# ishovkun/poroelasticity-dealii

Hardware: AMD Instinct MI355X
Metric: DoF-updates/sec in assemble+SpMV per fixed-stress iter (higher is better)
Workload: dtype f64

## Files before the change

poroelasticity_dealii_amd/csrc/common.hpp:

```cpp
#pragma once
#include <hip/hip_runtime.h>
#include <cstdint>
#include <cstdio>
#include <map>
#include <memory>
#include <type_traits>
#include <stdexcept>
#include <string>
#include <list>
#include <vector>
#include "../../include/poroel_hip.h"
#include "fdm_tables.hpp"
#include "cell_field.hpp"

namespace poro {

#define PORO_HIP(x)                                                                                   \
  do { hipError_t e_ = (x); if (e_ != hipSuccess) throw poro::Error(std::string(#x) + " -> " + hipGetErrorString(e_)); } while (0)

template <class T> struct DevBuf {
  T *p = nullptr; size_t n = 0;
  DevBuf() = default; DevBuf(const DevBuf &) = delete; DevBuf &operator=(const DevBuf &) = delete;
  ~DevBuf() { release(); }
  void release() { if (p) (void)hipFree(p); p = nullptr; n = 0; }
// ... 319 lines not shown
void p_residual_stencil(hipStream_t s, int dim, const BoxDev &box, double kappa, const double *t, const double *p, const double *src, double *R);
void p_stencil_apply_var(hipStream_t s, int dim, const BoxDev &box, double a, const double *kap, int ncomp, const double *x, double *y);
void p_residual_stencil_var(hipStream_t s, int dim, const BoxDev &box, const double *kap, int ncomp, const double *t, const double *p, const double *src, double *R);

struct KronCheb { const double *g = nullptr; double *znew = nullptr; double omega = 0; const uint8_t *cls = nullptr; const double *tab = nullptr;
                  double *side_lo = nullptr, *side_hi = nullptr; };
bool kron_supported(int dim, int k_u);
void kron_prepare_device();
BoxCoupling box_coupling(int dim, int k_u, const BoxDev &box);
void box_rhs_u(hipStream_t s, int dim, const BoxCoupling &B, double alpha, const double *p, const double *lift, const double *neu, const uint8_t *mask, double *rhs,
               const uint8_t *flags = nullptr );
int64_t box_rhs_u_flag_count(int64_t n_u);
void box_rhs_u_flags(hipStream_t s, const double *lift, const double *neu, int64_t n_u, uint8_t *flags );
void box_asm_u_matrix(hipStream_t s, int dim, int k_u, const BoxDev &box, const double *Ke, const CsrDev &A, const uint8_t *mask, double *val);
void box_proj_rhs(hipStream_t s, int dim, const BoxCoupling &B, const double *u, int n_comp, const int32_t *tensor_components, double *const *rhs);
void fdm_window_batch(hipStream_t s, double *grid, double *dense, double *dense_self, int self, bool to_block, const FdmWindow *win, int n_peers, int n_planes_pad, int64_t C, int64_t grid_stride, int64_t blk);
void fdm_window(hipStream_t s, double *dst, const double *src, bool to_block, int n_planes, int n_planes_pad, int64_t C, int64_t ncols_valid, int64_t grid_stride, int64_t grid_col0, int64_t grid_plane0);
void fdm_transform(hipStream_t s, const double *T, int n_l, int64_t SI, int64_t n_outer, const double *in, double *out, const FdmScale *scale);
void q1_line_factor(hipStream_t s, int dim, int nw, const FdmScalar &F, int nl, double a, const double *coef, double *inv);
void q1_line_solve(hipStream_t s, int dim, int nw, const FdmScalar &F, int nl, double a, bool fixed_lo, bool fixed_hi, const double *coef, const double *inv, const double *in, double *out);
void fdm_apply(hipStream_t s, const FdmScalar &F, double a, const double k[3], const double *g, double *z, double *t1, double *t2);
void fdmu_upload_dir(FdmuDir &D, const LineTables &T, bool single, bool split);
void fdmu_apply(hipStream_t s, const FdmU &F, const double *g, double *z, void *t1, void *t2, int stage);
void fdmu_window(hipStream_t s, double *dst, const double *src, bool to_block, int ncomp, int n_planes, int n_planes_pad, int64_t C, int64_t ncols_valid,
                 int64_t grid_stride, int64_t grid_planes, int64_t grid_col0, int64_t grid_plane0);
void fdmu_lines(hipStream_t s, const FdmU &F, const FdmuDir *last_dir, int64_t C, int64_t col0, int64_t ncol_valid, void *in, void *out);
struct FdmuLineArgs { int nl, n0; int64_t ncol; const double *coef; const double *lam0[3], *lam1[3]; int fixed[3][2]; };
void fdmu_line_factor(hipStream_t s, int ku, int ncomp, const FdmuLineArgs &a, double *fac );
void fdmu_line_solve(hipStream_t s, int ku, int ncomp, const FdmuLineArgs &a, const double *fac, double *v );
bool fdmo_usable(int dim, const int nn[3]);
void fdmo_init(FdmOct &O, const int nn[3], const double coef[3][3], hipStream_t s);
void fdmo_init_slab(FdmOct &O, const int nn[3], const double coef[3][3], int rank, const std::vector<int> &node_layers, bool has_upper, hipStream_t s);
void fdmo_init_per_direction(FdmOct &O, const int nn[3], const double coef[3][3], const FdmFormDecision &D, hipStream_t s);
void fdmo_upload_dir(FdmOct &O, int comp, int dir, const LineTables &T);
void fdmo_finalize(FdmOct &O);
void fdmo_apply(hipStream_t s, const FdmOct &O, const double *g_oct, double *z_oct, double *scratch_oct, const PcgScalars *gate = nullptr, hipEvent_t *ev  = nullptr,
                double *gz_part  = nullptr,
                int precision  = PORO_FDM_FP64,
                const PcgStopTest &stop = PcgStopTest{} );
bool fdmo_scalar_usable(int dim, const int nn[3]);
void fdmo_scalar_init(FdmOct &O, const int nn[3], hipStream_t s);
void fdmo_scalar_upload_dir(FdmOct &O, int dir, const LineTables &T);
void fdmo_scalar_apply(hipStream_t s, FdmOct &O, double a, double kappa, const double *g, double *z, const PcgScalars *gate = nullptr);
void fdmo_scalar_apply_many(hipStream_t s, FdmOct &O, double a, double kappa, int nb, const double *const *g, double *const *z, const PcgScalars *gate = nullptr);
void la_residual_norms_many(hipStream_t s, int nb, const double *const *y, const double *const *b, int64_t n, double *partials, const uint8_t *mask = nullptr);
void fdmo_scalar_init_slab(FdmOct &O, const int nn[3], int rank, const std::vector<int> &node_layers, hipStream_t s);
void fdmo_scalar_slab_pass(hipStream_t s, FdmOct &O, int pass, double a, double kappa, const double *in, double *out);
bool fdmo_planar_usable(int dim, const int nn[3]);
void fdmo_init_planar(FdmOct &O, const int nn[3], const double coef[3][3], hipStream_t s, bool split = true );
void fdmo_upload_dir_planar(FdmOct &O, int comp, int dir, const LineTables &T);
void fdmo_apply_planar(hipStream_t s, const FdmOct &O, const double *g_q, double *z_q, const PcgScalars *gate = nullptr, const PcgStopTest &stop = PcgStopTest{} );
void fdmo_from_nodal(hipStream_t s, const FdmOct &O, const double *v_nodal, double *q_oct);
void fdmo_to_nodal(hipStream_t s, const FdmOct &O, const double *r_oct, double *v_nodal);
void fdmo_init_residual(hipStream_t s, const FdmOct &O, double *g_oct, const double *Ax, const double *b, const uint8_t *inert);
void fdmo_first_direction(hipStream_t s, const FdmOct &O, double *d, const double *g_oct, const double *z_oct, double *partials );
void fdmo_update_g(hipStream_t s, const FdmOct &O, PcgScalars *sc, int parity, double *g_oct, const double *h, const uint8_t *inert, const double *partials_dh, double *partials_out , const double *red = nullptr);
void fdmo_update_d(hipStream_t s, const FdmOct &O, PcgScalars *sc, int parity, int it, double *x, double *d, const double *z_oct, const double *partials_in , const double *red = nullptr,
                   bool gz_from_pass = false ,
                   bool stream_x = false ,
                   bool decided = false ,
                   bool gg_stored = false );
void fdmo_dot_owned(hipStream_t s, const FdmOct &O, const double *a_oct, const double *b_oct, double *partials, const PcgScalars *gate);
void fdmo_slab_pass(hipStream_t s, const FdmOct &O, int pass , const double *in, double *out, const PcgScalars *gate, hipEvent_t e0 = nullptr, hipEvent_t e1 = nullptr);
void fdmo_slab_scatter_pack(hipStream_t s, const FdmOct &O, const PcgScalars *gate);
int kron_apply(hipStream_t s, const MfArgs &a, const double *x, double *y, bool constrained, int n_cus, double *dot_partials = nullptr, hipEvent_t ev0 = nullptr, hipEvent_t ev1 = nullptr,
               const PcgScalars *pcg = nullptr ,
               const KronCheb *cheb = nullptr );
void kron_fix_constrained(hipStream_t s, const MfArgs &a, const double *x, double *y, double *dot_partials, int slot_base);
void kron_lm_prepare_device();
int kron_lm_apply(hipStream_t s, const MfArgs &a, const double *planes, const double *x, double *y, bool constrained, int n_cus, double *dot_partials = nullptr, hipEvent_t ev0 = nullptr,
                  hipEvent_t ev1 = nullptr, const PcgScalars *pcg = nullptr);
void hyb_gather(hipStream_t s, int dim, int64_t n_box_nodes, const int64_t *inj, const double *x, double *x_box);
struct HybCombine { int64_t n_box_nodes, n_removed, n_chunks; const int64_t *inj; const uint8_t *touched; const int32_t *removed_cells, *slot, *chunk_cls; const int64_t *nodes;
                    const double *x_box, *y_box; double *V; };
void hyb_combine(hipStream_t s, const MfArgs &box, const double *Ke_t, bool constrained, const HybCombine &h, double *y);

}
```

poroelasticity_dealii_amd/csrc/ctx.hip:

```cpp
#include <dlfcn.h>
#include <rccl/rccl.h>
#include <algorithm>
#include <array>
#include <chrono>
#include <cmath>
#include <cstdlib>
#include <cstring>
#include <functional>
#include <thread>
#include <unordered_map>
#include "common.hpp"
#include "ctx_internal.hpp"

using namespace poro;
using namespace poro::ctx_detail;

namespace {
void lifting_from_wh(poro_ctx *c) {
  la_fill(c->stream, c->lift_u.p, 0.0, c->n_u);
  la_axpy(c->stream, c->lift_u.p, -1.0, c->wh_u.p, c->n_u);
}

void throw_unless_close(poro_ctx *c, double *a, const double *b, int64_t n, double rel_tol, const char *what) {
  hipStream_t s = c->stream;
// ... 204 lines not shown
        exchange_planes(c, c->cheb_side_lo.p, c->cheb_side_hi.p, plane);
      }
      la_cheb_fix_planes(s, zn, zj, g, kc.side_lo, c->comm.recv_lo.p, kc.side_hi, c->comm.recv_hi.p, sys.diag, omega, c->n_u, plane);
    }
    if (dp) la_dot_partials(s, g, zn, n_own, dp);
    return dp != nullptr;
  };
  auto step_fused = [&](const double *g, double *zj, double *zn, double omega, double *dp, const PcgScalars *pstate) {
    const KronCheb kc = cheb_update(g, zn, omega);
    if (dp) PORO_HIP(hipMemsetAsync(dp, 0, kMaxPartials * sizeof(double), s));
    const int slots = fused_kernel(zj, kc, dp, pstate);
    return dp && slots > 0;
  };
  auto step_unfused = [&](const double *g, double *zj, double *zn, double omega, double *dp) {
    sys.apply(zj, c->cheb_t.p, nullptr);
    la_cheb_step(s, zn, zj, g, c->cheb_t.p, sys.diag, omega, c->n_u, n_own, dp);
    return dp != nullptr;
  };
  sys.prec.z = z_u(c);
  sys.prec.gated = fuse;
  sys.prec.applications = m;
  sys.z1.out = (m % 2 == 0) ? sys.prec.z : c->cheb_z.p;
  sys.z1.scale = 1.0 / roots[0];
  sys.prec.fn = [&](const double *g, double *z, const PrecCall &call) {
    Timed tm(c, "precondition_u_chebyshev");
    double *X[2] = {(m % 2 == 0) ? z : c->cheb_z.p, (m % 2 == 0) ? c->cheb_z.p : z};
    if (!call.z1_ready) la_cheb_first(s, X[0], g, sys.diag, 1.0 / roots[0], c->n_u);
    bool dot_done = false;
    for (int j = 1; j <= m; ++j) {
      const double omega = 1.0 / roots[j];
      double *zj = X[(j - 1) & 1], *zn = X[j & 1];
      double *dp = j == m ? call.gz_partials : nullptr;
      if (fuse_multi) dot_done = step_fused_slabs(g, zj, zn, omega, dp);
      else if (fuse) dot_done = step_fused(g, zj, zn, omega, dp, call.gate);
      else dot_done = step_unfused(g, zj, zn, omega, dp);
      ++c->cheb_applies;
    }
    return dot_done ? GzLeft::in_partials : GzLeft::nowhere;
  };
  const int rc = pcg(c, sys, opts, info);
  finish_u(c, true);
  return rc;
}

int solve_u_fdm(poro_ctx *c, const poro_solver_opts *opts, poro_solve_info *info) {
  build_fdm_u(c);
  const FdmOct *oct = c->fdm_oct.built ? &c->fdm_oct : nullptr;
  const bool separate_gz = std::getenv("PORO_FDMO_SEPARATE_GZ") != nullptr;
  const bool shared = oct && !oct->slab.on && !oct->planar && std::getenv("PORO_FDMO_SEPARATE_BUFFERS") == nullptr;
  if (shared) c->timers["fdm_u_shared_buffers"].enqueued++;
  if (oct && oct->per_dir) c->timers["fdm_u_per_direction_form"].enqueued++;
  const int precision = oct && oct->per_dir ? PORO_FDM_FP64 : c->fdm_precision;
  double *const scratch = shared && precision != PORO_FDM_FP32 ? nullptr : c->fdm_oct.t.p;
  KrylovSystem sys = krylov_u(c, c->dir_mask.p, false, c->pcg_hint_fdm_u);
  if (shared) sys.h = c->fdm_oct.z.p;
  sys.oct.form = oct;
  sys.oct.stream_x = shared;
  sys.prec.z = c->wz_u.p;
  sys.prec.gated = oct != nullptr;
  sys.prec.decides_stop = oct && !oct->slab.on;
  sys.prec.fn = [&](const double *g, double *z, const PrecCall &call) {
    if (!oct) {
      fdm_precondition_u(c, g, z);
      return GzLeft::nowhere;
    }
    const bool gz = call.gz_partials && !separate_gz;
    return fdm_precondition_u_form(c, g, z, call.gate, precision, scratch, gz ? c->fdm_oct.gz_part.p : nullptr, call.stop) ? GzLeft::in_octant_form : GzLeft::nowhere;
  };
  const int rc = pcg(c, sys, opts, info);
  finish_u(c, false);
  return rc;
}

int solve_u_two_level(poro_ctx *c, const poro_solver_opts *opts, poro_solve_info *info) {
  if (!two_level_supported(c)) throw Error("PORO_PREC_TWO_LEVEL needs poro_desc.coarse (a refinement of a uniform box whose Dirichlet conditions cover whole faces)");
  const double om = opts->omega > 0 ? opts->omega : 1.0;
  KrylovSystem sys = krylov_u(c, c->cons_u.inert.p, false, c->pcg_hint_u);
  sys.prec.z = z_u(c);
  sys.prec.fn = [&](const double *g, double *z, const PrecCall &) {
    two_level_precondition_u(c, g, z, om);
    return GzLeft::nowhere;
  };
  const int rc = pcg(c, sys, opts, info);
  finish_u(c, true);
  return rc;
}

int solve_u_jacobi(poro_ctx *c, const poro_solver_opts *opts, poro_solve_info *info) {
  const int rc = pcg(c, krylov_u(c, c->cons_u.inert.p, true, c->pcg_hint_u), opts, info);
  finish_u(c, true);
  return rc;
}

struct Q1System {
  double a, kappa;
  const double *val;
  const double *dinv;
  DevBuf<double> *ilu;
  bool *ilu_valid;
  double *x;
  const double *b;
  int *hint;
  const uint8_t *inert;
  const uint8_t *inert_fdm = nullptr;
  Q1Set set = Q1Set::free_ends;
  Q1Set coarse_set = Q1Set::free_ends;
  const double *kap = nullptr;
  int kap_ncomp = 0;
  int perm_kind = 0;
  bool distribute_inhom = true;
// ... 806 lines not shown
```

poroelasticity_dealii_amd/csrc/ctx_internal.hpp:

```cpp
#pragma once
#include <rccl/rccl.h>
#include <functional>
#include <string>
#include <vector>
#include "common.hpp"
#include "whole_faces.hpp"
#include "fdm_tables.hpp"

namespace poro {
namespace ctx_detail {

extern thread_local std::string g_err;
inline int ipow(int b, int e) { int r = 1; while (e--) r *= b; return r; }
template <class F> int guarded(F &&f) {
  try { return f(); }
  catch (const std::exception &e) { g_err = e.what(); return -1; }
}
template <class F> void for_each_colour(poro_ctx *c, F &&fn) {
  for (size_t k = 0; k + 1 < c->color_off.size(); ++k)
    fn(c->color_cells.p + c->color_off[k], c->color_off[k + 1] - c->color_off[k]);
}

struct Rccl {
  void *lib = nullptr;
// ... 34 lines not shown
  ~EventPair() { c->event_pool.push_back(e0); c->event_pool.push_back(e1); }
  EventPair(const EventPair &) = delete; EventPair &operator=(const EventPair &) = delete;
};
void post_and_wait(poro_ctx *c, const double *dev_src, int n, const PcgScalars *sc = nullptr);

void setup_general_partition(poro_ctx *c, const poro_desc *d);
void exchange_planes(poro_ctx *c, const double *send_lo, const double *send_hi, int64_t plane);
void exchange_add(poro_ctx *c, double *v, int64_t n, int64_t plane);
void allreduce_sum(poro_ctx *c, double *dev, int n);
void allreduce_sum_vec(poro_ctx *c, double *dev, int64_t n, const char *timer);
int64_t owned(poro_ctx *c, int64_t n, int64_t plane);
AsmArgs asm_args(poro_ctx *c);
MfArgs mf_args(poro_ctx *c);
void mf_operator(poro_ctx *c, const double *x, double *y, bool constrained);
void mfg_operator(poro_ctx *c, const double *x, double *y, bool constrained);
void build_spatial_cells(poro_ctx *c);
void sync_moduli_planes(poro_ctx *c);
void hybrid_enable(poro_ctx *c);
void hybrid_operator(poro_ctx *c, const double *x, double *y, bool constrained);
void count_mfg_launches(poro_ctx *c, int n);
double *vec(poro_ctx *c, int which);
int64_t vec_len(poro_ctx *c, int which);
bool is_u_vec(int which);
bool apply_A_u(poro_ctx *c, const double *x, double *y, int mode, double *dot_partials = nullptr, bool fix_rows = true, const PcgScalars *pcg_state = nullptr,
               bool exchange = true );

typedef std::function<bool(const double *x, double *y, double *dh_partials)> ApplyFn;
struct PrecCall {
  const PcgScalars *gate = nullptr;
  double *gz_partials = nullptr;
  bool z1_ready = false;
  PcgStopTest stop;
};
enum class GzLeft { nowhere, in_partials , in_octant_form  };
typedef std::function<GzLeft(const double *g, double *z, const PrecCall &)> PrecFn;

struct KrylovSystem {
  int64_t n = 0, plane = 0;
  double *x = nullptr; const double *b = nullptr;
  ApplyFn apply;
  DiagVec diag;
  const uint8_t *inert = nullptr;
  double *g = nullptr, *d = nullptr, *h = nullptr;
  int cg1_set = 0;
  int *hint = nullptr;
  struct { PrecFn fn;
           double *z = nullptr;
           bool gated = false;
           bool decides_stop = false;
           int applications = 0;
  } prec;
  struct { const FdmOct *form = nullptr;
           bool stream_x = false;
  } oct;
  struct { double *out = nullptr; double scale = 0; } z1;
};
int pcg(poro_ctx *c, const KrylovSystem &sys, const poro_solver_opts *opts, poro_solve_info *info);
double dot_host(poro_ctx *c, const double *a, const double *b, int64_t n);
int pcg_csr_sweeps(poro_ctx *c, CsrDev &A, const double *val, DevBuf<double> &lu, bool &lu_valid, KrylovSystem &sys, const poro_solver_opts *opts, poro_solve_info *info);
double estimate_lmax_u(poro_ctx *c, const KrylovSystem &sys);

bool fdm_p_supported(poro_ctx *c);
bool fdm_pj_supported(poro_ctx *c);
enum class Q1Set { free_ends, fixed_ends };
inline FdmQ1 &q1_set(poro_ctx *c, Q1Set which) { return which == Q1Set::fixed_ends ? c->q1_fixed : c->q1_free; }
void build_fdm_q1(poro_ctx *c, Q1Set which);
int slab_layout(poro_ctx *c, SlabLayout &L, int nodes_per_cell, int64_t ncol_total);
const char *prec_refusal(poro_ctx *c, int which_system, int prec, bool solving = false);
void alltoall_blocks(poro_ctx *c, double *send, double *recv, int64_t blk, bool self_in_place = false );
void setup_two_level(poro_ctx *c, const poro_desc *d);
bool two_level_supported(poro_ctx *c);
bool two_level_supported_p(poro_ctx *c);
bool two_level_supported_pj(poro_ctx *c);
void two_level_precondition_p(poro_ctx *c, double a, double kappa, const double *dinv, const double *g, double *z, double omega, const uint8_t *inert, Q1Set coarse_set = Q1Set::free_ends);
void two_level_precondition_u(poro_ctx *c, const double *g, double *z, double omega);
bool fdm_precondition_u_form(poro_ctx *c, const double *g_form, double *z_form, const PcgScalars *gate, int precision, double *scratch, double *gz_part = nullptr, const PcgStopTest &stop = PcgStopTest{});
void fdm_precondition_u_nodal(poro_ctx *c, const double *g, double *z, int precision);
void fdm_precondition_p(poro_ctx *c, double a, const double k[3], const double *g, double *z, Q1Set which = Q1Set::free_ends);
void fdm_precondition_p_layered(poro_ctx *c, double a, const double *g, double *z, Q1Set which = Q1Set::free_ends);
void analyse_fdm_u(poro_ctx *c);
void build_fdm_u(poro_ctx *c);
FdmuLineArgs fdmu_line_args(poro_ctx *c);
void release_fdm_u(poro_ctx *c);
void fdm_precondition_u(poro_ctx *c, const double *g, double *z);

void validate_rows(const int64_t *ptr, const int32_t *col, const double *weight, int64_t n_rows, int64_t n_cols, const std::string &what);
void build_kelly_tables(poro_ctx *c);

void setup(poro_ctx *c, const poro_desc *d);
void sync_source_vector(poro_ctx *c);

}
}
```

poroelasticity_dealii_amd/csrc/ctx_pcg.hip:

```cpp
#include <dlfcn.h>
#include <rccl/rccl.h>
#include <algorithm>
#include <array>
#include <chrono>
#include <cmath>
#include <cstdlib>
#include <cstring>
#include <functional>
#include <thread>
#include <unordered_map>
#include "common.hpp"
#include "ctx_internal.hpp"

using namespace poro;
using namespace poro::ctx_detail;

namespace poro {
namespace ctx_detail {
static int expected_iterations(const int *hint, bool cheap_overshoot) {
  if (!hint || hint[0] <= 0) return 0;
  const int expect = std::max(hint[1] > 0 ? 2 * hint[0] - hint[1] : hint[0], hint[0] / 2);
  return std::min(expect, cheap_overshoot ? hint[0] + std::max(2, hint[0] / 4) : hint[0]);
}
template <class State> static int finish_solve(const KrylovSystem &sys, const State &hs, int64_t own, double seconds, poro_solve_info *info) {
// ... 13 lines not shown
  double *x = sys.x, *g = sys.g, *d = sys.d, *sv = sys.h, *w = wbuf.p, *z = precond ? sys.prec.z : zbuf.p;
  if (!z) throw Error("pcg: explicit preconditioner without a z vector");
  const bool jacobi = opts->preconditioner == PORO_PREC_JACOBI;
  Cg1State *st = c->cg1_state.p; double *part = c->partials.p, *red = c->red.p;
  EventPair ev(c); PORO_HIP(hipEventRecord(ev.e0, s));
  sys.apply(x, w, nullptr);
  pcg_init_residual(s, g, w, sys.b, sys.inert, n);
  la_fill(s, d, 0.0, n); la_fill(s, sv, 0.0, n);
  double *z1_out = sys.z1.out; double z1_scale = sys.z1.scale;
  if (jacobi && !precond) { z1_out = z; z1_scale = 1.0; }
  Cg1State hs{};
  int enq = 0;
  const int expect = expected_iterations(sys.hint, false);
  auto next_batch = [&](int done_its) { const int left = expect - 4 - done_its; return left >= 4 ? std::min(32, left) : 2; };
  int batch = expect > 0 ? next_batch(0) : 1;
  while (true) {
    for (int k = 0; k < batch; ++k) {
      if (precond) { PrecCall call; call.z1_ready = enq > 0 && sys.z1.out != nullptr; (void)precond(g, z, call); }
      else if (jacobi) { if (enq == 0) la_cheb_first(s, z, g, sys.diag, 1.0, n); }
      else la_copy(s, z, g, n);
      sys.apply(z, w, nullptr);
      cg1_dots(s, g, z, w, enq == 0 ? sys.b : nullptr, n_own, part);
      pcg_scalars_sum(s, part, 4, red);
      allreduce_sum(c, red, 4);
      cg1_scalars(s, st, red, enq == 0 ? 1 : 0, opts->abs_tol, opts->rel_tol, opts->max_iter, opts->stop_rule);
      cg1_update(s, st, d, sv, x, g, z, w, sys.diag, sys.inert, z1_out, z1_scale, n);
      ++enq;
    }
    PORO_HIP(hipMemcpyAsync(&hs, st, sizeof(hs), hipMemcpyDeviceToHost, s)); PORO_HIP(hipStreamSynchronize(s));
    if (hs.done) break;
    if (expect > 0) batch = next_batch(enq); else if (batch < 8) batch *= 2;
  }
  PORO_HIP(hipEventRecord(ev.e1, s)); PORO_HIP(hipEventSynchronize(ev.e1));
  float ms = 0; PORO_HIP(hipEventElapsedTime(&ms, ev.e0, ev.e1));
  return finish_solve(sys, hs, hs.it + 2, ms * 1e-3, info);
}

int pcg(poro_ctx *c, const KrylovSystem &sys, const poro_solver_opts *opts, poro_solve_info *info) {
  static const bool two_reductions = std::getenv("PORO_TWO_REDUCTION_CG") != nullptr;
  const FdmOct *oct = sys.oct.form;
  const bool multi = c->comm.multi();
  if (multi && !two_reductions && !oct) return pcg_single_reduction(c, sys, opts, info);
  hipStream_t s = c->stream;
  const PrecFn &precond = sys.prec.fn;
  const int prec = opts->preconditioner == PORO_PREC_JACOBI ? 1 : 0;
  if (oct && (!precond || multi != oct->slab.on)) throw Error("pcg: the octant form needs an explicit preconditioner (one rank: octants, slab partition: quadrants)");
  const int64_t n = sys.n, n_own = owned(c, n, sys.plane);
  double *x = sys.x, *d = sys.d, *h = sys.h, *g = oct ? oct->g.p : sys.g, *zbuf = oct ? oct->z.p : sys.prec.z;
  if (precond && !zbuf) throw Error("pcg: explicit preconditioner without a z vector");
  double *part = c->partials.p, *red = c->red.p; PcgScalars *sc = c->scal.p;
  double *part_dh = part + 3 * (size_t)kMaxPartials;
  const auto t_start = std::chrono::steady_clock::now();
  sys.apply(x, h, nullptr);
  if (oct) fdmo_init_residual(s, *oct, g, h, sys.b, sys.inert); else pcg_init_residual(s, g, h, sys.b, sys.inert, n);
  if (opts->stop_rule != PORO_STOP_REDUCTION) la_dot_partials(s, sys.b, sys.b, n_own, part);
  if (precond) (void)precond(g, zbuf, PrecCall{});
  if (oct) fdmo_first_direction(s, *oct, d, g, zbuf, part + kMaxPartials); else pcg_first_direction(s, d, g, sys.diag, zbuf, prec, n, n_own, part + kMaxPartials);
  pcg_scalars_sum(s, part, 3, red);
  allreduce_sum(c, red, 3);
  pcg_scalars_start(s, sc, red, opts->abs_tol, opts->rel_tol, opts->max_iter, opts->stop_rule);
  PORO_HIP(hipMemsetAsync(part_dh, 0, kMaxPartials * sizeof(double), s));
  PcgScalars hs{};
  int it = 0;
  const bool cheap_overshoot = !precond || sys.prec.gated;
  const int expect = expected_iterations(sys.hint, cheap_overshoot);
  const bool small = n <= 400000;
  int batch = expect > 0 ? (cheap_overshoot ? std::min(expect, 256) : std::max(1, expect - 1)) : (precond && !cheap_overshoot && !small ? 1 : 4);
  PrecCall call;
  call.gate = sys.prec.gated ? sc : nullptr; call.gz_partials = part + kMaxPartials; call.z1_ready = sys.z1.out != nullptr;
  const bool stop_in_prec = oct && !multi && sys.prec.gated && sys.prec.decides_stop && std::getenv("PORO_PCG_FINAL_PREC") == nullptr;
  const int stop_per_wave = std::getenv("PORO_PCG_STOP_PER_WAVE") != nullptr ? 1 : 0;
  const bool gg_stored = stop_in_prec && std::getenv("PORO_PCG_GG_RESUM") == nullptr;
  while (true) {
    for (int k = 0; k < batch; ++k) {
      ++it;
      if (stop_in_prec) call.stop = PcgStopTest{sc, part, it, stop_per_wave};
      if (!sys.apply(d, h, part_dh)) pcg_dot_dh(s, sc, d, h, n_own, part_dh);
      if (multi) { pcg_scalars_sum(s, part_dh, 1, red); allreduce_sum(c, red, 1); }
      if (oct) fdmo_update_g(s, *oct, sc, (it - 1) & 1, g, h, sys.inert, part_dh, part, multi ? red : nullptr);
      else pcg_update_g_fused(s, sc, (it - 1) & 1, g, h, sys.diag, zbuf, sys.z1.out, sys.z1.scale, prec, n, n_own, part_dh, multi ? red : nullptr, part);
      const GzLeft gz = precond ? precond(g, zbuf, call) : GzLeft::in_partials;
      if (gz == GzLeft::nowhere) {
        if (oct && multi) fdmo_dot_owned(s, *oct, g, zbuf, call.gz_partials, call.gate);
        else la_dot_partials(s, g, zbuf, oct ? oct->n_oct : n_own, call.gz_partials, call.gate);
      }
      if (multi) { pcg_scalars_sum(s, part, 2, red + 1); allreduce_sum(c, red + 1, 2); }
      if (oct) fdmo_update_d(s, *oct, sc, (it - 1) & 1, it, x, d, zbuf, part, multi ? red + 1 : nullptr, gz == GzLeft::in_octant_form, sys.oct.stream_x, stop_in_prec, gg_stored);
      else pcg_update_d_fused(s, sc, (it - 1) & 1, it, x, d, g, sys.diag, zbuf, prec, n, part, multi ? red + 1 : nullptr);
    }
    post_and_wait(c, nullptr, 0, sc); hs = c->mailbox->sc;
    if (hs.done || hs.finishing) break;
    if (expect > 0) batch = cheap_overshoot ? 3 : small ? 2 : 1;
    else if (cheap_overshoot && precond) batch = 4;
    else if (batch < 32) batch *= 2;
  }
  if (hs.stop) c->timers["fdm_u_final_prec_skipped"].enqueued++;
  return finish_solve(sys, hs, hs.it + 1, std::chrono::duration<double>(std::chrono::steady_clock::now() - t_start).count(), info);
}

void build_ssor_levels(poro_ctx *c, CsrDev &A) {
  if (A.ssor.built) return;
  std::vector<int64_t> rp(A.n + 1); std::vector<int32_t> col(A.nnz);
  PORO_HIP(hipMemcpy(rp.data(), A.rp.p, (A.n + 1) * sizeof(int64_t), hipMemcpyDeviceToHost)); PORO_HIP(hipMemcpy(col.data(), A.col.p, A.nnz * sizeof(int32_t), hipMemcpyDeviceToHost));
  auto levels = [&](bool fwd, DevBuf<int32_t> &rows_dev, std::vector<int64_t> &off) {
    std::vector<int32_t> lvl(A.n, 0); int maxl = 0;
    if (fwd) for (int64_t r = 0; r < A.n; ++r) { int l = 0; for (int64_t j = rp[r]; j < rp[r + 1] && col[j] < r; ++j) l = std::max(l, lvl[col[j]] + 1); lvl[r] = l; maxl = std::max(maxl, l); }
    else for (int64_t r = A.n - 1; r >= 0; --r) { int l = 0; for (int64_t j = rp[r + 1] - 1; j >= rp[r] && col[j] > r; --j) l = std::max(l, lvl[col[j]] + 1); lvl[r] = l; maxl = std::max(maxl, l); }
    off.assign(maxl + 2, 0);
    for (int64_t r = 0; r < A.n; ++r) off[lvl[r] + 1]++;
    for (int l = 0; l <= maxl; ++l) off[l + 1] += off[l];
    std::vector<int32_t> rows(A.n); std::vector<int64_t> pos(off.begin(), off.end() - 1);
    for (int64_t r = 0; r < A.n; ++r) rows[pos[lvl[r]]++] = (int32_t)r;
    rows_dev.upload(rows);
  };
  levels(true, A.ssor.fwd_rows, A.ssor.fwd_off); levels(false, A.ssor.bwd_rows, A.ssor.bwd_off);
  A.ssor.built = true;
}
double dot_host(poro_ctx *c, const double *a, const double *b, int64_t n) {
  la_dot_partials(c->stream, a, b, n, c->partials.p); la_reduce_finish(c->stream, c->partials.p, 1, c->red.p, 0);
  allreduce_sum(c, c->red.p, 1);
  post_and_wait(c, c->red.p, 1);
  return c->mailbox->vals[0];
}
static int pcg_host(poro_ctx *c, const KrylovSystem &sys, const poro_solver_opts *opts, poro_solve_info *info) {
  hipStream_t s = c->stream;
  const int64_t n = sys.n, n_own = n;
  double *x = sys.x, *g = sys.g, *d = sys.d, *h = sys.h; const double *b = sys.b;
  const auto t0 = std::chrono::steady_clock::now();
  int64_t applies = 0; int it = 0, conv = 0;
  sys.apply(x, g, nullptr); ++applies;
  la_axpy(s, g, -1.0, b, n);
  double res = std::sqrt(dot_host(c, g, g, n_own)); const double res0 = res;
  const double tol = std::max(opts->abs_tol, opts->rel_tol * (opts->stop_rule == PORO_STOP_REDUCTION ? res0 : std::sqrt(dot_host(c, b, b, n_own))));
  if (res <= tol) conv = 1;
  else {
    (void)sys.prec.fn(g, h, PrecCall{});
    la_fill(s, d, 0.0, n); la_axpy(s, d, -1.0, h, n);
    double gh = dot_host(c, g, h, n_own);
    while (true) {
      ++it;
// ... 81 lines not shown
```

poroelasticity_dealii_amd/csrc/kernels_fdmo.hip:

```cpp
#include "common.hpp"
#include "fdm_tables.hpp"
#include "device_reduce.hpp"
#include <hip/hip_ext.h>
#include <cmath>
#include <cstdlib>
#include <limits>
#include <mutex>
#include <set>
#include <type_traits>

namespace poro {
namespace {

typedef double v4d __attribute__((ext_vector_type(4)));
typedef float v4f __attribute__((ext_vector_type(4)));

struct OctDims { int nx, ny, nz, hx, hy, hz, hxp; int64_t co; int no, own_z, nc; int split; int part[8]; };

__device__ __forceinline__ void bfly_fwd(double (&v)[8], const bool (&centre)[3]) {
#pragma unroll
  for (int bit = 0; bit < 3; ++bit) {
    const int m = 1 << bit;
#pragma unroll
    for (int i = 0; i < 8; ++i) if (!(i & m)) {
// ... 116 lines not shown
  const double alpha = sc->gh2[parity] / dh;
  double gg = 0;
  for (int64_t t_ = (int64_t)blockIdx.x * kBlock + threadIdx.x; t_ < NC * (D.co / 2); t_ += (int64_t)gridDim.x * kBlock) {
    const int64_t pr = t_ / NC; const int c = (int)(t_ - NC * pr); const int64_t idx = 2 * pr;
    const OctPos<PD> P0(D, idx), P1(D, idx + 1);
    double w0[8], w1[8];
    const bool on0 = P0.valid && !(inert && inert[P0.node[0] * NC + c]), on1 = P1.valid && !(inert && inert[P1.node[0] * NC + c]);
#pragma unroll
    for (int m = 0; m < 8; ++m) { w0[m] = on0 ? h[P0.node[m] * NC + c] : 0.0; w1[m] = on1 ? h[P1.node[m] * NC + c] : 0.0; }
    bfly_fwd(w0, P0.centre); bfly_fwd(w1, P1.centre);
    double s0 = 0, s1 = 0;
#pragma unroll
    for (int o = 0; o < 8; ++o) if (part_on<PD>(D, o)) {
      double2 *gp = reinterpret_cast<double2 *>(g + (int64_t)(c * D.no + part_at<PD>(D, o)) * D.co + idx);
      double2 gv = *gp;
      gv.x = fma(alpha, w0[o], gv.x); gv.y = fma(alpha, w1[o], gv.y);
      *gp = gv; s0 = fma(gv.x, gv.x, s0); s1 = fma(gv.y, gv.y, s1);
    }
    if (P0.own) gg = fma(P0.weight, s0, fma(P1.weight, s1, gg));
  }
  gg = block_sum(gg, sh);
  store_partial(partials_out, gg);
  if (blockIdx.x == 0 && threadIdx.x == 0) { sc->dh = dh; sc->alpha = alpha; }
}
template <int NC, bool XNT, bool PD> __global__ void __launch_bounds__(kBlock) k_fdmo_update_d(OctDims D, PcgScalars *sc, int parity, int it, double *__restrict__ x, double *__restrict__ d, const double *__restrict__ z, int64_t n_u, const double *partials_in, const double *red,
                                                                            const double *gz_part, int gz_n, int decided ) {
  __shared__ double sh[5];
  if (sc->done) return;
  const double gg = red ? red[0] : decided == 2 ? sc->gg : sum_partials(partials_in, sh);
  const double res = sqrt(gg), gh_old = sc->gh2[parity], alpha = sc->alpha;
  const int stop = decided ? sc->stop : res <= sc->tol ? 1 : it >= sc->max_iter ? 2 : 0;
  const bool conv = stop == 1, fail = stop == 2, no_z = decided && stop;
  const double gz = no_z ? 0.0 : red ? red[1] : gz_part ? sum_partials(gz_part, sh, gz_n) : sum_partials(partials_in + kMaxPartials, sh);
  if (blockIdx.x == 0 && threadIdx.x == 0) { sc->gg = gg; if (!no_z) sc->gz = gz; sc->res = res; sc->it = it; }
  if (conv || fail) {
    for (int64_t i = (int64_t)blockIdx.x * kBlock + threadIdx.x; i < n_u; i += (int64_t)gridDim.x * kBlock) x[i] = fma(alpha, d[i], x[i]);
    if (blockIdx.x == 0 && threadIdx.x == 0) { sc->converged = conv ? 1 : 0; sc->finishing = 1; }
    return;
  }
  const double beta = gz / gh_old;
  PORO_OCT_LOOP(D) {
    PORO_OCT_DECODE(D)
    double w[8];
#pragma unroll
    for (int o = 0; o < 8; ++o) w[o] = part_on<PD>(D, o) ? z[(int64_t)(c * D.no + part_at<PD>(D, o)) * D.co + idx] : 0.0;
    bfly_bwd(w, P.centre);
#pragma unroll
    for (int m = 0; m < 8; ++m) if (P.live[m]) {
      const int64_t dof = P.node[m] * NC + c;
      const double dv = d[dof], xv = XNT ? __builtin_nontemporal_load(&x[dof]) : x[dof];
      if (XNT) __builtin_nontemporal_store(fma(alpha, dv, xv), &x[dof]); else x[dof] = fma(alpha, dv, xv);
      d[dof] = fma(beta, dv, -w[m]);
    }
  }
  if (blockIdx.x == 0 && threadIdx.x == 0) { sc->beta = beta; sc->gh2[parity ^ 1] = gz; }
}

__global__ void __launch_bounds__(kBlock) k_fdmo_dot_owned(OctDims D, const double *__restrict__ a, const double *__restrict__ b, double *partials, const PcgScalars *gate) {
  __shared__ double sh[5];
  if (gate && (gate->done | gate->finishing)) return;
  const int64_t per = (int64_t)D.own_z * D.hxp * D.hy;
  const int nblk = D.nc * D.no, share = gridDim.x / nblk, blk = blockIdx.x / max(share, 1), sub = blockIdx.x - blk * share;
  double acc = 0;
  if (share > 0 && blk < nblk) {
    const double2 *__restrict__ a2 = reinterpret_cast<const double2 *>(a + blk * D.co), *__restrict__ b2 = reinterpret_cast<const double2 *>(b + blk * D.co);
    for (int64_t e = (int64_t)sub * kBlock + threadIdx.x; e < per / 2; e += (int64_t)share * kBlock) { const double2 u = a2[e], v = b2[e]; acc = fma(u.x, v.x, fma(u.y, v.y, acc)); }
  }
  acc = block_sum(acc, sh);
  store_partial(partials, acc);
}

struct SlabGeo { int cw, nchunk, cps, chunk_total, rank, my_chunks, hzg, ng, np; int64_t scols, pl, co; };
__global__ void __launch_bounds__(256) k_fdmo_slab_scatter_pack(SlabGeo S, int rows, const int64_t *__restrict__ row_out, const int32_t *__restrict__ row_kz,
                                                                  const double *__restrict__ tz, double *__restrict__ buf, const PcgScalars *gate) {
  if (gate && (gate->done | gate->finishing)) return;
  const int per_row = S.my_chunks * S.cw, total = rows * per_row;
  for (int e = blockIdx.x * 256 + threadIdx.x; e < total; e += gridDim.x * 256) {
    const int row = e / per_row, col = e - row * per_row, cl = col / S.cw, j = col - cl * S.cw;
    const int kz = row_kz[row];
    if (S.np == 1) { buf[row_out[row] + col] = tz[((int64_t)cl * S.hzg + kz) * S.cw + j]; continue; }
    const int mz = S.ng - 1 - kz, kh = min(kz, mz);
    const double a = tz[((int64_t)(2 * cl) * S.hzg + kh) * S.cw + j], b = tz[((int64_t)(2 * cl + 1) * S.hzg + kh) * S.cw + j];
    buf[row_out[row] + col] = kz == mz ? a : (kz < mz ? a + b : a - b);
  }
}

struct OctPass {
  int mode;
  int R, C;
  int kk1, kk2;
  int nblk;
  int64_t co_stride, blk_stride, row_stride;
  int bit1, bit2;
  int pl;
  const void *T1[3][2], *T2[3][2];
  const double *lam_z[3][2]; double cz[3]; const double *bxy;
  const double *in_blk[3]; double *out_blk[3]; int use_in_off, use_out_off;
  int bxy_cmul;
  int no_shift;
  int slab_z , chunk0, chunk_total, nchunk;
  int slab_io, store_planes, ng, scols, col_unit, rank; float inv_scols; int64_t dest_stride, recv_off; const int64_t *row_in;
  int vec2;
  int per_dir, bitz;
  double *gz_part;
  const PcgScalars *gate;
  PcgStopTest stop;
// ... 972 lines not shown
  O.co_stride = (int64_t)O.hxp * O.h[1]; O.n_oct = 2 * O.no * O.co_stride;
  O.g.alloc(O.n_oct); O.z.alloc(O.n_oct); O.t.alloc(2 * O.n_oct);
  O.g.zero(s); O.z.zero(s); O.t.zero(s);
}
void fdmo_upload_dir_planar(FdmOct &O, int comp, int dir, const LineTables &T) {
  const int nn = T.n; const std::vector<double> &S = T.S, &lam = T.lam;
  if (nn != O.n[dir]) throw Error("fdmo_upload_dir_planar: line length mismatch");
  if (O.no == 1) {
    std::vector<double> F((size_t)nn * nn, 0.0), lp((size_t)nn + 16, std::numeric_limits<double>::infinity());
    for (int m = 0; m < nn; ++m) { if (!(lam[m] < 1e300)) continue; for (int k = 0; k < nn; ++k) F[(size_t)m * nn + k] = S[(size_t)k * nn + m]; lp[m] = lam[m]; }
    O.h_lam[comp][dir][0] = lp; O.fwd[comp][dir][0].upload(F); O.lam[comp][dir][0].upload(lp);
    return;
  }
  const int h = (nn + 1) / 2;
  if (!T.parity) throw Error("fdmo_upload_dir_planar: tables whose modes are not all even or odd");
  const std::vector<int> *const grp[2] = {&T.even, &T.odd};
  for (int p = 0; p < 2; ++p) {
    std::vector<double> F((size_t)h * h, 0.0), lp((size_t)h + 16, std::numeric_limits<double>::infinity());
    const std::vector<int> &g = *grp[p]; const int ng = (int)g.size();
    for (int m = 0; m < ng; ++m) { for (int k = 0; k < h; ++k) F[(size_t)m * h + k] = S[(size_t)k * nn + g[m]]; lp[m] = lam[g[m]]; }
    O.h_lam[comp][dir][p] = lp; O.fwd[comp][dir][p].upload(F); O.lam[comp][dir][p].upload(lp);
  }
}
void fdmo_apply_planar(hipStream_t s, const FdmOct &O, const double *g, double *z, const PcgScalars *gate, const PcgStopTest &stop) {
  const int hx = O.h[0], hy = O.h[1], hxp = O.hxp; const int64_t co = O.co_stride;
  double *t1 = O.t.p, *t2 = O.t.p + O.n_oct;
  const int no = O.no, nb = 2 * no;
  if (stop.gg_part && stop.sc != gate) throw Error("fdmo_apply_planar: a stopping test without the gate of its solve");
  Gemm2D G{}; G.nb = nb; G.gate = gate; G.rsC = hxp; G.stop = stop;
  auto launch = [&](bool ak, bool bk) {
    const dim3 grid((unsigned)(((G.M + 63) / 64) * ((G.N + 63) / 64)), (unsigned)nb);
    if (ak && bk) hipLaunchKernelGGL((k_fdmo_gemm2d<true, true>), grid, 256, 0, s, G);
    else if (ak) hipLaunchKernelGGL((k_fdmo_gemm2d<true, false>), grid, 256, 0, s, G);
    else hipLaunchKernelGGL((k_fdmo_gemm2d<false, false>), grid, 256, 0, s, G);
  };
  G.M = hy; G.N = hx; G.K = hx; G.rsA = hxp; G.csA = 1; G.rsB = 1; G.csB = hx; G.scale = 0;
  for (int b = 0; b < nb; ++b) { const int c = b / no, q = b % no; G.A[b] = g + (int64_t)b * co; G.B[b] = O.fwd[c][0][q & 1].p; G.C[b] = t1 + (int64_t)b * co; }
  launch(true, true);
  G.stop = PcgStopTest{};
  G.M = hy; G.N = hx; G.K = hy; G.rsA = hy; G.csA = 1; G.rsB = hxp; G.csB = 1; G.scale = 1;
  for (int b = 0; b < nb; ++b) { const int c = b / no, q = b % no; G.A[b] = O.fwd[c][1][q >> 1].p; G.B[b] = t1 + (int64_t)b * co; G.C[b] = t2 + (int64_t)b * co;
                                G.lamM[b] = O.lam[c][1][q >> 1].p; G.lamN[b] = O.lam[c][0][q & 1].p; G.cM[b] = O.coef[c][1]; G.cN[b] = O.coef[c][0]; }
  launch(true, false);
  G.rsA = 1; G.csA = hy; G.scale = 0;
  for (int b = 0; b < nb; ++b) { G.B[b] = t2 + (int64_t)b * co; G.C[b] = t1 + (int64_t)b * co; }
  launch(false, false);
  G.M = hy; G.N = hx; G.K = hx; G.rsA = hxp; G.csA = 1; G.rsB = hx; G.csB = 1;
  for (int b = 0; b < nb; ++b) { const int c = b / no, q = b % no; G.A[b] = t1 + (int64_t)b * co; G.B[b] = O.fwd[c][0][q & 1].p; G.C[b] = z + (int64_t)b * co; }
  launch(true, false);
}

void fdmo_from_nodal(hipStream_t s, const FdmOct &O, const double *v, double *q) { PORO_OCT_LAUNCH(k_fdmo_from_nodal, O, v, (const uint8_t *)nullptr, q); }
void fdmo_to_nodal(hipStream_t s, const FdmOct &O, const double *r, double *v) { PORO_OCT_LAUNCH(k_fdmo_to_nodal, O, r, v); }
void fdmo_init_residual(hipStream_t s, const FdmOct &O, double *g, const double *Ax, const double *b, const uint8_t *inert) { PORO_OCT_LAUNCH(k_fdmo_init_residual, O, g, Ax, b, inert); }
void fdmo_first_direction(hipStream_t s, const FdmOct &O, double *d, const double *g, const double *z, double *partials) { PORO_OCT_LAUNCH(k_fdmo_first_direction, O, d, g, z, partials); }
void fdmo_update_g(hipStream_t s, const FdmOct &O, PcgScalars *sc, int parity, double *g, const double *h, const uint8_t *inert, const double *partials_dh, double *partials_out, const double *red) {
  static const bool single = std::getenv("PORO_FDMO_UPDATE_G_SINGLE") != nullptr;
  if (single) PORO_OCT_LAUNCH(k_fdmo_update_g, O, sc, parity, g, h, inert, partials_dh, partials_out, red);
  else PORO_OCT_LAUNCH(k_fdmo_update_g2, O, sc, parity, g, h, inert, partials_dh, partials_out, red);
}
template <int NC, bool XNT, bool PD> static void launch_update_d(hipStream_t s, const FdmOct &O, PcgScalars *sc, int parity, int it, double *x, double *d, const double *z, const double *partials_in, const double *red, bool gz_from_pass, int decided) {
  hipLaunchKernelGGL((k_fdmo_update_d<NC, XNT, PD>), oct_grid(O.co_stride, NC), kBlock, 0, s, dims_of(O), sc, parity, it, x, d, z, (int64_t)O.nc * O.n[0] * O.n[1] * O.n[2], partials_in, red,
                     gz_from_pass ? (const double *)O.gz_part.p : (const double *)nullptr, gz_from_pass ? O.gz_n : 0, decided);
}
void fdmo_update_d(hipStream_t s, const FdmOct &O, PcgScalars *sc, int parity, int it, double *x, double *d, const double *z, const double *partials_in, const double *red, bool gz_from_pass, bool stream_x, bool decided, bool gg_stored) {
  const int dec = decided ? (gg_stored && !red ? 2 : 1) : 0;
  if (O.nc == 2) launch_update_d<2, false, false>(s, O, sc, parity, it, x, d, z, partials_in, red, gz_from_pass, dec);
  else if (O.per_dir && stream_x) launch_update_d<3, true, true>(s, O, sc, parity, it, x, d, z, partials_in, red, gz_from_pass, dec);
  else if (O.per_dir) launch_update_d<3, false, true>(s, O, sc, parity, it, x, d, z, partials_in, red, gz_from_pass, dec);
  else if (stream_x) launch_update_d<3, true, false>(s, O, sc, parity, it, x, d, z, partials_in, red, gz_from_pass, dec);
  else launch_update_d<3, false, false>(s, O, sc, parity, it, x, d, z, partials_in, red, gz_from_pass, dec);
}

}
```

Before: 24.40 billion.

## Add row-tiled LDS form of the octant update_d kernel for coalesced nodal access

Adds a row-based variant of the FDM octant update_d kernel. Each block stages one (y,z) row of octant data in LDS, runs the backward butterfly there, and then updates the nodal x and d entries in contiguous row order, instead of scattering per position. It is turned on by default for single-rank, non-per-direction, non-fp32 octant forms with hx up to 128, and init_residual is switched to a matching launch. The goal is more coalesced global memory traffic for d and x. The cost is extra LDS use and two syncthreads per row, and the grid is capped at kMaxPartials blocks.

```diff
diff --git a/poroelasticity_dealii_amd/csrc/common.hpp b/poroelasticity_dealii_amd/csrc/common.hpp
--- a/poroelasticity_dealii_amd/csrc/common.hpp
+++ b/poroelasticity_dealii_amd/csrc/common.hpp
@@ -395,14 +395,16 @@
 void fdmo_apply_planar(hipStream_t s, const FdmOct &O, const double *g_q, double *z_q, const PcgScalars *gate = nullptr, const PcgStopTest &stop = PcgStopTest{} );
 void fdmo_from_nodal(hipStream_t s, const FdmOct &O, const double *v_nodal, double *q_oct);
 void fdmo_to_nodal(hipStream_t s, const FdmOct &O, const double *r_oct, double *v_nodal);
-void fdmo_init_residual(hipStream_t s, const FdmOct &O, double *g_oct, const double *Ax, const double *b, const uint8_t *inert);
+bool fdmo_row_form_usable(const FdmOct &O);
+void fdmo_init_residual(hipStream_t s, const FdmOct &O, double *g_oct, const double *Ax, const double *b, const uint8_t *inert, bool rows = false);
 void fdmo_first_direction(hipStream_t s, const FdmOct &O, double *d, const double *g_oct, const double *z_oct, double *partials );
 void fdmo_update_g(hipStream_t s, const FdmOct &O, PcgScalars *sc, int parity, double *g_oct, const double *h, const uint8_t *inert, const double *partials_dh, double *partials_out , const double *red = nullptr);
 void fdmo_update_d(hipStream_t s, const FdmOct &O, PcgScalars *sc, int parity, int it, double *x, double *d, const double *z_oct, const double *partials_in , const double *red = nullptr,
                    bool gz_from_pass = false ,
                    bool stream_x = false ,
                    bool decided = false ,
-                   bool gg_stored = false );
+                   bool gg_stored = false ,
+                   bool rows = false);
 void fdmo_dot_owned(hipStream_t s, const FdmOct &O, const double *a_oct, const double *b_oct, double *partials, const PcgScalars *gate);
 void fdmo_slab_pass(hipStream_t s, const FdmOct &O, int pass , const double *in, double *out, const PcgScalars *gate, hipEvent_t e0 = nullptr, hipEvent_t e1 = nullptr);
 void fdmo_slab_scatter_pack(hipStream_t s, const FdmOct &O, const PcgScalars *gate);
diff --git a/poroelasticity_dealii_amd/csrc/ctx.hip b/poroelasticity_dealii_amd/csrc/ctx.hip
--- a/poroelasticity_dealii_amd/csrc/ctx.hip
+++ b/poroelasticity_dealii_amd/csrc/ctx.hip
@@ -280,10 +280,14 @@
   if (oct && oct->per_dir) c->timers["fdm_u_per_direction_form"].enqueued++;
   const int precision = oct && oct->per_dir ? PORO_FDM_FP64 : c->fdm_precision;
   double *const scratch = shared && precision != PORO_FDM_FP32 ? nullptr : c->fdm_oct.t.p;
+  const char *const vform = std::getenv("PORO_FDMO_VECTOR_FORM");
+  const bool rows = oct && fdmo_row_form_usable(*oct) && precision != PORO_FDM_FP32 && !(vform && std::string(vform) == "positions");
+  if (rows) c->timers["fdm_u_row_form"].enqueued++;
   KrylovSystem sys = krylov_u(c, c->dir_mask.p, false, c->pcg_hint_fdm_u);
   if (shared) sys.h = c->fdm_oct.z.p;
   sys.oct.form = oct;
   sys.oct.stream_x = shared;
+  sys.oct.rows = rows;
   sys.prec.z = c->wz_u.p;
   sys.prec.gated = oct != nullptr;
   sys.prec.decides_stop = oct && !oct->slab.on;
diff --git a/poroelasticity_dealii_amd/csrc/ctx_internal.hpp b/poroelasticity_dealii_amd/csrc/ctx_internal.hpp
--- a/poroelasticity_dealii_amd/csrc/ctx_internal.hpp
+++ b/poroelasticity_dealii_amd/csrc/ctx_internal.hpp
@@ -110,6 +110,7 @@
   } prec;
   struct { const FdmOct *form = nullptr;
            bool stream_x = false;
+           bool rows = false;
   } oct;
   struct { double *out = nullptr; double scale = 0; } z1;
 };
diff --git a/poroelasticity_dealii_amd/csrc/ctx_pcg.hip b/poroelasticity_dealii_amd/csrc/ctx_pcg.hip
--- a/poroelasticity_dealii_amd/csrc/ctx_pcg.hip
+++ b/poroelasticity_dealii_amd/csrc/ctx_pcg.hip
@@ -89,7 +89,7 @@
   double *part_dh = part + 3 * (size_t)kMaxPartials;
   const auto t_start = std::chrono::steady_clock::now();
   sys.apply(x, h, nullptr);
-  if (oct) fdmo_init_residual(s, *oct, g, h, sys.b, sys.inert); else pcg_init_residual(s, g, h, sys.b, sys.inert, n);
+  if (oct) fdmo_init_residual(s, *oct, g, h, sys.b, sys.inert, sys.oct.rows); else pcg_init_residual(s, g, h, sys.b, sys.inert, n);
   if (opts->stop_rule != PORO_STOP_REDUCTION) la_dot_partials(s, sys.b, sys.b, n_own, part);
   if (precond) (void)precond(g, zbuf, PrecCall{});
   if (oct) fdmo_first_direction(s, *oct, d, g, zbuf, part + kMaxPartials); else pcg_first_direction(s, d, g, sys.diag, zbuf, prec, n, n_own, part + kMaxPartials);
@@ -122,7 +122,7 @@
         else la_dot_partials(s, g, zbuf, oct ? oct->n_oct : n_own, call.gz_partials, call.gate);
       }
       if (multi) { pcg_scalars_sum(s, part, 2, red + 1); allreduce_sum(c, red + 1, 2); }
-      if (oct) fdmo_update_d(s, *oct, sc, (it - 1) & 1, it, x, d, zbuf, part, multi ? red + 1 : nullptr, gz == GzLeft::in_octant_form, sys.oct.stream_x, stop_in_prec, gg_stored);
+      if (oct) fdmo_update_d(s, *oct, sc, (it - 1) & 1, it, x, d, zbuf, part, multi ? red + 1 : nullptr, gz == GzLeft::in_octant_form, sys.oct.stream_x, stop_in_prec, gg_stored, sys.oct.rows);
       else pcg_update_d_fused(s, sc, (it - 1) & 1, it, x, d, g, sys.diag, zbuf, prec, n, part, multi ? red + 1 : nullptr);
     }
     post_and_wait(c, nullptr, 0, sc); hs = c->mailbox->sc;
diff --git a/poroelasticity_dealii_amd/csrc/kernels_fdmo.hip b/poroelasticity_dealii_amd/csrc/kernels_fdmo.hip
--- a/poroelasticity_dealii_amd/csrc/kernels_fdmo.hip
+++ b/poroelasticity_dealii_amd/csrc/kernels_fdmo.hip
@@ -192,6 +192,81 @@
       if (XNT) __builtin_nontemporal_store(fma(alpha, dv, xv), &x[dof]); else x[dof] = fma(alpha, dv, xv);
       d[dof] = fma(beta, dv, -w[m]);
     }
+  }
+  if (blockIdx.x == 0 && threadIdx.x == 0) { sc->beta = beta; sc->gh2[parity ^ 1] = gz; }
+}
+
+constexpr int kRowBatch = 4;
+struct OctRow {
+  int ky, kz, my, mz, nlive; bool cy, cz; int64_t oct0;
+  __device__ __forceinline__ OctRow(const OctDims &D, int r) {
+    ky = r % D.hy; kz = r / D.hy; my = D.ny - 1 - ky; mz = D.nz - 1 - kz;
+    cy = my == ky; cz = mz == kz;
+    nlive = (cy ? 1 : 2) * (cz ? 1 : 2); oct0 = (int64_t)r * D.hxp;
+  }
+  __device__ __forceinline__ int slot(int q) const { const int ys = (q & 1) && !cy, zs = (q & 2) && !cz; return ys + (zs ? (cy ? 1 : 2) : 0); }
+  __device__ __forceinline__ int64_t row_dof(const OctDims &D, int s) const {
+    const int yb = cy ? 0 : (s & 1), zb = cy ? (s & 1) : (s >> 1);
+    return (((int64_t)(zb ? mz : kz) * D.ny + (yb ? my : ky)) * D.nx) * 3;
+  }
+};
+struct OctAt { int64_t g; int l, kx; __device__ __forceinline__ OctAt(const OctDims &D, const OctRow &R, int i) { const int hp = D.hxp >> 1, b = i / hp, j = i - b * hp; kx = 2 * j; l = b * D.hxp + kx; g = (int64_t)b * D.co + R.oct0 + kx; } };
+__device__ __forceinline__ int64_t row_dof_at(const OctDims &D, const OctRow &R, int i) { const int L = 3 * D.nx, s = i / L; return R.row_dof(D, s) + (i - s * L); }
+template <class T, class Get, class Put> __device__ __forceinline__ void row_batches(int n, Get get, Put put) {
+  for (int i0 = threadIdx.x; i0 < n; i0 += kRowBatch * kBlock) {
+    T v[kRowBatch];
+#pragma unroll
+    for (int u = 0; u < kRowBatch; ++u) if (i0 + u * kBlock < n) v[u] = get(i0 + u * kBlock);
+#pragma unroll
+    for (int u = 0; u < kRowBatch; ++u) if (i0 + u * kBlock < n) put(i0 + u * kBlock, v[u]);
+  }
+}
+struct RowUnit {
+  int c, kx, mx; bool centre[3];
+  __device__ __forceinline__ RowUnit(const OctDims &D, const OctRow &R, int u) { c = u / D.hx; kx = u - c * D.hx; mx = D.nx - 1 - kx; centre[0] = mx == kx; centre[1] = R.cy; centre[2] = R.cz; }
+  __device__ __forceinline__ bool live(int m) const { return !((m & 1) && centre[0]) && !((m & 2) && centre[1]) && !((m & 4) && centre[2]); }
+  __device__ __forceinline__ int nod(const OctDims &D, const OctRow &R, int m) const { return R.slot(m >> 1) * 3 * D.nx + 3 * ((m & 1) ? mx : kx) + c; }
+  __device__ __forceinline__ int oct(const OctDims &D, int o) const { return (c * 8 + o) * D.hxp + kx; }
+};
+#define PORO_ROW_TILES(D) extern __shared__ __attribute__((aligned(16))) double row_tile_[]; double *const oct = row_tile_, *const nod = row_tile_ + 24 * (D).hxp;
+#define PORO_ROW_LOOP(D) for (int r_ = blockIdx.x; r_ < (D).hy * (D).hz; r_ += gridDim.x)
+
+template <bool XNT> __global__ void __launch_bounds__(kBlock) k_fdmo_update_d_rows(OctDims D, PcgScalars *sc, int parity, int it, double *__restrict__ x, double *__restrict__ d, const double *__restrict__ z, int64_t n_u, const double *partials_in, const double *red,
+                                                                                   const double *gz_part, int gz_n, int decided) {
+  PORO_ROW_TILES(D)
+  __shared__ double sh[5];
+  if (sc->done) return;
+  const double gg = red ? red[0] : decided == 2 ? sc->gg : sum_partials(partials_in, sh);
+  const double res = sqrt(gg), gh_old = sc->gh2[parity], alpha = sc->alpha;
+  const int stop = decided ? sc->stop : res <= sc->tol ? 1 : it >= sc->max_iter ? 2 : 0;
+  const bool conv = stop == 1, fail = stop == 2, no_z = decided && stop;
+  const double gz = no_z ? 0.0 : red ? red[1] : gz_part ? sum_partials(gz_part, sh, gz_n) : sum_partials(partials_in + kMaxPartials, sh);
+  if (blockIdx.x == 0 && threadIdx.x == 0) { sc->gg = gg; if (!no_z) sc->gz = gz; sc->res = res; sc->it = it; }
+  if (conv || fail) {
+    for (int64_t i = (int64_t)blockIdx.x * kBlock + threadIdx.x; i < n_u; i += (int64_t)gridDim.x * kBlock) x[i] = fma(alpha, d[i], x[i]);
+    if (blockIdx.x == 0 && threadIdx.x == 0) { sc->converged = conv ? 1 : 0; sc->finishing = 1; }
+    return;
+  }
+  const double beta = gz / gh_old;
+  PORO_ROW_LOOP(D) {
+    const OctRow R(D, r_);
+    row_batches<double2>(12 * D.hxp, [&](int i) { return *reinterpret_cast<const double2 *>(z + OctAt(D, R, i).g); }, [&](int i, double2 v) { *reinterpret_cast<double2 *>(oct + OctAt(D, R, i).l) = v; });
+    __syncthreads();
+    for (int u = threadIdx.x; u < 3 * D.hx; u += kBlock) {
+      const RowUnit U(D, R, u);
+      double w[8];
+#pragma unroll
+      for (int o = 0; o < 8; ++o) w[o] = oct[U.oct(D, o)];
+      bfly_bwd(w, U.centre);
+#pragma unroll
+      for (int m = 0; m < 8; ++m) if (U.live(m)) nod[U.nod(D, R, m)] = w[m];
+    }
+    __syncthreads();
+    row_batches<double2>(R.nlive * 3 * D.nx, [&](int i) { const int64_t dof = row_dof_at(D, R, i); return make_double2(d[dof], XNT ? __builtin_nontemporal_load(&x[dof]) : x[dof]); }, [&](int i, double2 dx) {
+      const int64_t dof = row_dof_at(D, R, i);
+      if (XNT) __builtin_nontemporal_store(fma(alpha, dx.x, dx.y), &x[dof]); else x[dof] = fma(alpha, dx.x, dx.y);
+      d[dof] = fma(beta, dx.x, -nod[i]);
+    });
   }
   if (blockIdx.x == 0 && threadIdx.x == 0) { sc->beta = beta; sc->gh2[parity ^ 1] = gz; }
 }
@@ -1270,7 +1345,14 @@
 
 void fdmo_from_nodal(hipStream_t s, const FdmOct &O, const double *v, double *q) { PORO_OCT_LAUNCH(k_fdmo_from_nodal, O, v, (const uint8_t *)nullptr, q); }
 void fdmo_to_nodal(hipStream_t s, const FdmOct &O, const double *r, double *v) { PORO_OCT_LAUNCH(k_fdmo_to_nodal, O, r, v); }
-void fdmo_init_residual(hipStream_t s, const FdmOct &O, double *g, const double *Ax, const double *b, const uint8_t *inert) { PORO_OCT_LAUNCH(k_fdmo_init_residual, O, g, Ax, b, inert); }
+bool fdmo_row_form_usable(const FdmOct &O) { return O.built && O.nc == 3 && O.no == 8 && !O.per_dir && !O.slab.on && !O.planar && O.h[0] <= 128; }
+static int row_grid(const FdmOct &O) { return std::min(O.h[1] * O.h[2], kMaxPartials); }
+static size_t row_lds(const FdmOct &O) { return (size_t)(24 * O.hxp + 4 * 3 * O.n[0]) * sizeof(double); }
+static void check_row_form(const FdmOct &O) { if (!fdmo_row_form_usable(O)) throw Error("fdmo: the row form of the vector kernels serves the single-rank octant form only"); }
+void fdmo_init_residual(hipStream_t s, const FdmOct &O, double *g, const double *Ax, const double *b, const uint8_t *inert, bool rows) {
+  if (rows) { check_row_form(O); hipLaunchKernelGGL((k_fdmo_init_residual<3, false>), (int)((3 * O.co_stride + kBlock - 1) / kBlock), kBlock, 0, s, dims_of(O), g, Ax, b, inert); }
+  else PORO_OCT_LAUNCH(k_fdmo_init_residual, O, g, Ax, b, inert);
+}
 void fdmo_first_direction(hipStream_t s, const FdmOct &O, double *d, const double *g, const double *z, double *partials) { PORO_OCT_LAUNCH(k_fdmo_first_direction, O, d, g, z, partials); }
 void fdmo_update_g(hipStream_t s, const FdmOct &O, PcgScalars *sc, int parity, double *g, const double *h, const uint8_t *inert, const double *partials_dh, double *partials_out, const double *red) {
   static const bool single = std::getenv("PORO_FDMO_UPDATE_G_SINGLE") != nullptr;
@@ -1281,8 +1363,17 @@
   hipLaunchKernelGGL((k_fdmo_update_d<NC, XNT, PD>), oct_grid(O.co_stride, NC), kBlock, 0, s, dims_of(O), sc, parity, it, x, d, z, (int64_t)O.nc * O.n[0] * O.n[1] * O.n[2], partials_in, red,
                      gz_from_pass ? (const double *)O.gz_part.p : (const double *)nullptr, gz_from_pass ? O.gz_n : 0, decided);
 }
-void fdmo_update_d(hipStream_t s, const FdmOct &O, PcgScalars *sc, int parity, int it, double *x, double *d, const double *z, const double *partials_in, const double *red, bool gz_from_pass, bool stream_x, bool decided, bool gg_stored) {
+template <bool XNT> static void launch_update_d_rows(hipStream_t s, const FdmOct &O, PcgScalars *sc, int parity, int it, double *x, double *d, const double *z, const double *partials_in, const double *red, bool gz_from_pass, int decided) {
+  hipLaunchKernelGGL((k_fdmo_update_d_rows<XNT>), row_grid(O), kBlock, row_lds(O), s, dims_of(O), sc, parity, it, x, d, z, (int64_t)O.nc * O.n[0] * O.n[1] * O.n[2], partials_in, red,
+                     gz_from_pass ? (const double *)O.gz_part.p : (const double *)nullptr, gz_from_pass ? O.gz_n : 0, decided);
+}
+void fdmo_update_d(hipStream_t s, const FdmOct &O, PcgScalars *sc, int parity, int it, double *x, double *d, const double *z, const double *partials_in, const double *red, bool gz_from_pass, bool stream_x, bool decided, bool gg_stored, bool rows) {
   const int dec = decided ? (gg_stored && !red ? 2 : 1) : 0;
+  if (rows) {
+    check_row_form(O);
+    if (stream_x) launch_update_d_rows<true>(s, O, sc, parity, it, x, d, z, partials_in, red, gz_from_pass, dec); else launch_update_d_rows<false>(s, O, sc, parity, it, x, d, z, partials_in, red, gz_from_pass, dec);
+    return;
+  }
   if (O.nc == 2) launch_update_d<2, false, false>(s, O, sc, parity, it, x, d, z, partials_in, red, gz_from_pass, dec);
   else if (O.per_dir && stream_x) launch_update_d<3, true, true>(s, O, sc, parity, it, x, d, z, partials_in, red, gz_from_pass, dec);
   else if (O.per_dir) launch_update_d<3, false, true>(s, O, sc, parity, it, x, d, z, partials_in, red, gz_from_pass, dec);
```

Result: no change. 24.39 billion (-0.0%).
